# VladimirP1/rs-sync

Measured on AMD Instinct MI355X. Metric: ray-residuals/sec (PreSync sweep + Sync iter), 4096 frames x 2048 tracks, higher is better.
Workload: dtype f32

## Files before the change

### rs-sync_amd/csrc/kernels/sync64.hpp

```cpp
#pragma once

#pragma clang fp contract(off)

namespace {



struct Loss64Params {
    Rays64 rays;
    const FrameRec* frames;
    const uint32_t* sel;
    uint32_t n_sel;
    const d4* coef;
    int n_knots;
    double fs;
    const int32_t* kd;
    const double* fd;
    uint32_t n_delays;
    const uint32_t* grp;
    uint32_t n_grp;
    const double* M;
    const double* k;
    double* part_loss;
    double* part_grad;
// ... 462 lines not shown
            }
        } else {
        double ss = 0.0;
        if constexpr (RPT != 0) {
#pragma unroll
            for (int j = 0; j < RPT; ++j) {
                const double pm = p.simple_k ? sqrt(rs::dot(ev.P[j], ev.P[j])) : rs::dot(ev.P[j], Mv);
                ss = fma(pm, pm, ss);
            }
        } else {
            for (int j = 0; j < ev.rpt; ++j) {
                const size_t i = (size_t)j * kThreads + tid;
                const d3 Pj = d3{ev.gP[i], ev.gP[ev.g_rows + i], ev.gP[2 * (size_t)ev.g_rows + i]};
                const double pm = p.simple_k ? sqrt(rs::dot(Pj, Pj)) : rs::dot(Pj, Mv);
                ss = fma(pm, pm, ss);
            }
        }
        const double sw = wave_sum_f64(ss);
        if ((tid & 63) == 0) s_red[tid >> 6] = sw;
        __syncthreads();
        tot = s_red[0];
#pragma unroll
        for (int w = 1; w < NW; ++w) tot += s_red[w];
        }
        kk = clamp_k(100.0 / sqrt(tot));
        x[0] = Mv.x; x[1] = Mv.y; x[2] = Mv.z;
        if (tid == 0) {
            if (!p.simple_k) { st_m<SC1>(&p.M[3 * sf], x[0]); st_m<SC1>(&p.M[3 * sf + 1], x[1]); st_m<SC1>(&p.M[3 * sf + 2], x[2]); }
            st_m<SC1>(&p.k[sf], kk);
            if (p.init_h) st_m<SC1>(&p.init_h[sf], (int32_t)kInitNone);
        }
    } else {
        x[0] = m_x; x[1] = m_y; x[2] = m_z;
        kk = m_k;
    }
    if (mk_out) { mk_out[0] = x[0]; mk_out[1] = x[1]; mk_out[2] = x[2]; mk_out[3] = kk; }
    if (p.max_iters <= 0 || p.simple_k) return;
    ev.k2 = kk * kk;
    if constexpr (EMU4) {
        if ((size_t)N * 24u <= (size_t)p.win_bytes) {
            __syncthreads();
            __attribute__((address_space(3))) double* l = (__attribute__((address_space(3))) double*)reinterpret_cast<double*>(s_win);
            for (uint32_t row = tid; row < N; row += kThreads) {
                l[row] = ev.gP[row];
                l[N + row] = ev.gP[ev.g_rows + row];
                l[2 * N + row] = ev.gP[2 * (size_t)ev.g_rows + row];
            }
            __syncthreads();
            ev.lP = l;
            ev.n_lds = N;
        }
    }

    LbfgsHistLds hist{s_S, s_Y, s_inv_ys, s_rho, s_alpha};
    int best_not_last = 0;
    K3_T0();
    const int it = rs::lbfgs3(ev, hist, x, p.max_iters , p.reeval, &best_not_last);
    K3_ADD(12, 13);
    K3_FLUSH(ev);
    if (mk_out) { mk_out[0] = x[0]; mk_out[1] = x[1]; mk_out[2] = x[2]; }
    if (tid == 0) {
        st_m<SC1>(&p.M[3 * sf], x[0]); st_m<SC1>(&p.M[3 * sf + 1], x[1]); st_m<SC1>(&p.M[3 * sf + 2], x[2]);
        if (p.stats) {
            atomicAdd(&p.stats[0], (unsigned long long)it);
            atomicAdd(&p.stats[1], (unsigned long long)ev.evals);
            atomicAdd(&p.stats[2], (unsigned long long)best_not_last);
        }
        if (p.per_frame) {
            p.per_frame[2 * sf] = (uint32_t)it;
            p.per_frame[2 * sf + 1] = (uint32_t)ev.evals;
        }
        if (p.evals_out) p.evals_out[sf] = (uint32_t)ev.evals;
    }
}

template <int RPT, int NW>
__global__ __launch_bounds__(64 * NW, NW == 4 ? (RPT == 0 ? 2 : (RPT <= 8 ? 3 : (RPT <= 24 ? 2 : 1))) : (NW == 1 ? (RPT >= 8 ? 3 : 4) : 2)) void opt_motion64_kernel(Motion64Params p) {
    __shared__ MotionLds<NW> lds;
    extern __shared__ d4 s_motion_win[];
    opt_motion64_body<RPT, NW>(p, p.order ? p.order[blockIdx.x + p.slot0] : blockIdx.x + p.slot0, lds, s_motion_win, nullptr,
                               p.scratch0 + blockIdx.x);
}

__global__ __launch_bounds__(1024) void motion_order_kernel(const uint32_t* __restrict__ evals, const uint32_t* __restrict__ list,
                                                            uint32_t* __restrict__ order, uint32_t pos0, uint32_t count) {
    __shared__ uint32_t s_bin[256];
    for (uint32_t b = threadIdx.x; b < 256; b += blockDim.x) s_bin[b] = 0;
    __syncthreads();
    for (uint32_t i = threadIdx.x; i < count; i += blockDim.x) {
        const uint32_t e = evals[list[pos0 + i]];
        atomicAdd(&s_bin[e < 255u ? e : 255u], 1u);
    }
    __syncthreads();
    if (threadIdx.x == 0) {
        uint32_t at = 0;
        for (int b = 255; b >= 0; --b) {
            const uint32_t n = s_bin[b];
            s_bin[b] = at;
            at += n;
        }
    }
    __syncthreads();
    for (uint32_t i = threadIdx.x; i < count; i += blockDim.x) {
        const uint32_t s = list[pos0 + i];
        const uint32_t e = evals[s];
        const uint32_t pos = atomicAdd(&s_bin[e < 255u ? e : 255u], 1u);
        order[pos0 + pos] = s;
    }
}

struct Debug64Params {
    Rays64 rays;
    const FrameRec* frames;
    uint32_t fi;
    const d4* coef;
    int n_knots;
    double fs;
    int32_t kd;
    double fd;
    double* P;
    double* dP;
};

__global__ __launch_bounds__(kBlock) void debug_problem64_kernel(Debug64Params p) {
    __shared__ d4 s_win[4 * kWinMax];
    const FrameRec fr = p.frames[p.fi];
    Spline64 sp;
    sp.g = p.coef;
    sp.n = p.n_knots;
    sp.cap = kWinMax;
    sp.compact = 0;
    frame_window64(sp, s_win, fr, p.kd);
    __syncthreads();
    for (uint32_t row = blockIdx.x * kBlock + threadIdx.x; row < fr.n; row += gridDim.x * kBlock) {
        d3 P, dP;
        residual_row64<true>(sp, p.rays, (size_t)fr.off + row, fr.base_knot + p.kd, p.fd, P, dP);
        p.P[3 * row] = P.x; p.P[3 * row + 1] = P.y; p.P[3 * row + 2] = P.z;
        if (p.dP) { p.dP[3 * row] = dP.x * p.fs; p.dP[3 * row + 1] = dP.y * p.fs; p.dP[3 * row + 2] = dP.z * p.fs; }
    }
}

__global__ __launch_bounds__(64) void debug_math64_kernel(int op, const double* __restrict__ a, const double* __restrict__ b,
                                                          double* __restrict__ out, uint32_t n) {
    const uint32_t i = blockIdx.x * 64 + threadIdx.x;
    const double x = i < n ? a[i] : 0.0, y = (i < n && b) ? b[i] : 0.0;
    if (op == 4) {
        const double t = wave_sum_f64(x);
        if (threadIdx.x == 0) out[blockIdx.x] = t;
        return;
    }
    if (i >= n) return;
    if (op == 0) out[i] = x / y;
    else if (op == 1) out[i] = sqrt(x);
    else if (op == 2) { double rc; out[2 * i] = rs::log1p_rcp_f64(x, &rc); out[2 * i + 1] = rc; }
    else if (op == 5) out[i] = rs::div3_exact(x);
    else out[i] = fma(x, y, x);
}

}

#pragma clang fp contract(fast)
```

### rs-sync_amd/csrc/kernels/syncloop.hpp

```cpp
#pragma once

namespace {

constexpr int kMaxBt = 10, kHalfBt = 5;

struct SyncWin {
    double d, v;
    double x0;
    double l1, g1;
    int active, conv, hit, iters;
    int phase;
    int nf;
    int hit_prev;
};

struct SyncLoopParams {
    SyncWin* win;
    uint32_t n_win;
    uint32_t win0, win1;
    const double* part;
    uint32_t n_sel, rows;
    const uint32_t* chunk_off;
    const uint32_t* win_chunk_off;
    double* chunk_tmp;
    uint32_t chunk_stride;
    int32_t* mo_kd; double* mo_fd;
    int32_t* lg_kd; double* lg_fd;
    int32_t* tr_kd; double* tr_fd;
    double fs;
    double ts[11];
    double c_armijo, delay_b, search_center, search_radius;
    int it, max_outer;
    int nf_fixed;
    int nf_floor;
    double* ext_sums;
    int* n_active;
    double* trace;
};


__device__ __forceinline__ void split64_dev(double delay, double fs, int32_t* kd, double* fd) {
#pragma clang fp contract(off)
    if (delay != delay) { *kd = 0; *fd = delay; return; }
    const double D = delay * fs;
    const double kClamp = (double)(1 << 29);
    if (!(fabs(D) <= 1.79769313486231570e308)) { *kd = 0; *fd = 0.0; return; }
    const double fl = floor(D);
    if (fl > kClamp) { *kd = 1 << 29; *fd = 0.0; return; }
    if (fl < -kClamp) { *kd = -(1 << 29); *fd = 0.0; return; }
    *kd = (int32_t)fl;
    *fd = D - fl;
}

constexpr uint32_t kStageDoubles = 2048;
__device__ __forceinline__ void window_sums(const SyncLoopParams& p, uint32_t w, double* s_tot, double* s_stage) {
    const uint32_t c0 = p.win_chunk_off[w], c1 = p.win_chunk_off[w + 1], nc = c1 - c0;
    const uint32_t j_lo = p.chunk_off[c0], j_hi = p.chunk_off[c1], span = j_hi - j_lo;
    double* tmp = p.chunk_tmp + (size_t)w * (2 * kMaxBt) * p.chunk_stride;
    const bool staged = p.rows * span <= kStageDoubles;
    if (staged) {
        for (uint32_t e = threadIdx.x; e < p.rows * span; e += blockDim.x)
            s_stage[e] = p.part[(size_t)(e / span) * p.n_sel + j_lo + e % span];
        __syncthreads();
    }
    for (uint32_t e = threadIdx.x; e < p.rows * nc; e += blockDim.x) {
        const uint32_t r = e / nc, c = c0 + e % nc;
        double acc = 0.0;
        uint32_t j = p.chunk_off[c];
        const uint32_t j1 = p.chunk_off[c + 1];
        if (staged) {
            const double* row = s_stage + (size_t)r * span - j_lo;
            for (; j + 8 <= j1; j += 8) {
                double v[8];
#pragma unroll
                for (int q = 0; q < 8; ++q) v[q] = row[j + q];
#pragma unroll
                for (int q = 0; q < 8; ++q) acc += v[q];
            }
            for (; j < j1; ++j) acc += row[j];
        } else {
            const double* row = p.part + (size_t)r * p.n_sel;
            const uint32_t cnt = j1 - j;
            if (cnt <= 64) {
                double v[64];
#pragma unroll
                for (int q = 0; q < 64; ++q) v[q] = (uint32_t)q < cnt ? row[j + q] : 0.0;
#pragma unroll
                for (int q = 0; q < 64; ++q)
                    if ((uint32_t)q < cnt) acc += v[q];
            } else {
                for (; j < j1; ++j) acc += row[j];
            }
        }
        tmp[(size_t)r * p.chunk_stride + (c - c0)] = acc;
    }
    __syncthreads();
    for (uint32_t r = threadIdx.x; r < p.rows; r += blockDim.x) {
        const double* t = tmp + (size_t)r * p.chunk_stride;
        double acc = 0.0;
        uint32_t c = 0;
        for (; c + 16 <= nc; c += 16) {
            double v[16];
#pragma unroll
            for (int q = 0; q < 16; ++q) v[q] = t[c + q];
#pragma unroll
            for (int q = 0; q < 16; ++q) acc += v[q];
        }
        for (; c < nc; ++c) acc += t[c];
        s_tot[r] = acc;
    }
    __syncthreads();
}

__global__ __launch_bounds__(64) void sync_begin_kernel(SyncLoopParams p) {
#pragma clang fp contract(off)
    const uint32_t w = p.win0 + blockIdx.x * 64 + threadIdx.x;
    if (w >= p.win1) return;
    SyncWin& s = p.win[w];
    s.x0 = s.active ? s.d - p.delay_b * s.v : __builtin_nan("");
    split64_dev(s.active ? s.d : __builtin_nan(""), p.fs, &p.mo_kd[w], &p.mo_fd[w]);
    split64_dev(s.x0, p.fs, &p.lg_kd[w], &p.lg_fd[w]);
}

__device__ __forceinline__ bool trial_wanted(const SyncWin& s, int i) {
    if (!s.active) return false;
    return s.phase == 0 ? i < s.nf : i >= s.nf;
}

__device__ __forceinline__ void grad_decide(const SyncLoopParams& p, SyncWin& s, double l1, double g1) {
#pragma clang fp contract(off)
    if (s.active && s.phase == 0) {
        s.l1 = l1;
        s.g1 = g1;
        s.hit = -1;
        if (s.iters == 0 && !p.nf_fixed) {
            int i = 0;
            while (i < kMaxBt - 1 && p.ts[i] * fabs(s.g1) >= 1e-3) ++i;
            const int want = i + 2;
            s.nf = want < kHalfBt ? kHalfBt : (want > kMaxBt ? kMaxBt : want);
        }
    }
}
__device__ __forceinline__ void trial_delays(const SyncLoopParams& p, const SyncWin& s, int32_t* tr_kd, double* tr_fd, size_t stride) {
#pragma clang fp contract(off)
    for (int i = 0; i < kMaxBt; ++i) {
        const double td = trial_wanted(s, i) ? s.x0 - p.ts[i] * s.g1 : __builtin_nan("");
        split64_dev(td, p.fs, &tr_kd[(size_t)i * stride], &tr_fd[(size_t)i * stride]);
    }
}

__global__ __launch_bounds__(kBlock) void sync_sums_kernel(SyncLoopParams p) {
#pragma clang fp contract(off)
    __shared__ double s_tot[2 * kMaxBt];
    __shared__ double s_stage[kStageDoubles];
    const uint32_t w = blockIdx.x + p.win0;
    window_sums(p, w, s_tot, s_stage);
    for (uint32_t r = threadIdx.x; r < p.rows; r += blockDim.x) p.ext_sums[(size_t)r * p.n_win + w] = s_tot[r];
}
__device__ __forceinline__ void decision_sums(const SyncLoopParams& p, uint32_t w, double* s_tot, double* s_stage) {
    if (p.ext_sums) {
        for (uint32_t r = threadIdx.x; r < p.rows; r += blockDim.x) s_tot[r] = p.ext_sums[(size_t)r * p.n_win + w];
        __syncthreads();
    } else {
        window_sums(p, w, s_tot, s_stage);
    }
}

__global__ __launch_bounds__(kBlock) void sync_grad_kernel(SyncLoopParams p) {
#pragma clang fp contract(off)
    __shared__ double s_tot[2 * kMaxBt];
    __shared__ double s_stage[kStageDoubles];
    const uint32_t w = blockIdx.x + p.win0;
    decision_sums(p, w, s_tot, s_stage);
    if (threadIdx.x != 0) return;
    SyncWin& s = p.win[w];
    grad_decide(p, s, s_tot[0], s_tot[1]);
    trial_delays(p, s, p.tr_kd + w, p.tr_fd + w, p.n_win);
}

__device__ __forceinline__ void armijo(const SyncLoopParams& p, SyncWin& s, const double* lt, int b0, int b1) {
#pragma clang fp contract(off)
    if (!s.active || s.hit >= 0) return;
    const double m = s.g1 * s.g1;
    for (int i = b0; i < b1; ++i) {
        if (s.l1 - lt[i] >= p.ts[i] * p.c_armijo * m) {
            s.hit = i;
            break;
        }
    }
}

__device__ __forceinline__ bool step_decide(const SyncLoopParams& p, SyncWin& s, const double* lt, double* rows, size_t row_stride) {
#pragma clang fp contract(off)
    bool step_now = false;
    if (s.active) {
        if (s.phase == 0) {
            armijo(p, s, lt, 0, s.nf);
            if (s.hit >= 0 || s.nf >= kMaxBt) step_now = true;
            else s.phase = 1;
        } else {
            armijo(p, s, lt, s.nf, kMaxBt);
            step_now = true;
        }
    }
    if (step_now) {
        const double v = s.l1, g = s.g1;
        const double t = s.hit >= 0 ? p.ts[s.hit] : p.ts[kMaxBt];
        const int trials = s.hit >= 0 ? s.hit + 1 : kMaxBt;
        const double step = -t * g;
        s.v = p.delay_b * s.v + step;
        s.d += s.v;
        const double step_size = fabs(step);
        double* row = rows + (size_t)s.iters * row_stride;
        row[0] = s.d; row[1] = step; row[2] = v; row[3] = g; row[4] = t; row[5] = (double)trials;
        s.iters += 1;
        s.phase = 0;
        const int last = s.hit >= 0 ? s.hit : kMaxBt - 1;
        const int want = (last > s.hit_prev ? last : s.hit_prev) + 1;
        s.hit_prev = last;
        s.nf = p.nf_fixed ? p.nf_fixed : (want < p.nf_floor ? p.nf_floor : (want > kMaxBt ? kMaxBt : want));
        if (step_size < 1e-4) s.conv++; else s.conv = 0;
        bool stop = s.conv > 5;
        if (!stop && fabs(s.d - p.search_center) > p.search_radius) stop = true;
        if (stop || s.iters == p.max_outer) s.active = 0;
    }
    s.x0 = s.active ? s.d - p.delay_b * s.v : __builtin_nan("");
    return step_now;
}

__global__ __launch_bounds__(kBlock) void sync_step_kernel(SyncLoopParams p) {
#pragma clang fp contract(off)
    __shared__ double s_tot[2 * kMaxBt];
    __shared__ double s_stage[kStageDoubles];
    const uint32_t w = blockIdx.x + p.win0;
    decision_sums(p, w, s_tot, s_stage);
    if (threadIdx.x != 0) return;
    SyncWin& s = p.win[w];
    step_decide(p, s, s_tot, p.trace + (size_t)w * 6, (size_t)p.n_win * 6);
    if (s.active) atomicAdd(&p.n_active[p.it], 1);
    const bool go = s.active && s.phase == 0;
    split64_dev(go ? s.d : __builtin_nan(""), p.fs, &p.mo_kd[w], &p.mo_fd[w]);
    split64_dev(go ? s.x0 : __builtin_nan(""), p.fs, &p.lg_kd[w], &p.lg_fd[w]);
}

}
```

### rs-sync_amd/csrc/rssync_kernels.hip

```cpp
#include <hip/hip_runtime.h>

#include <dlfcn.h>

#include <algorithm>
#include <cmath>
#include <cstdio>
#include <cstdlib>
#include <cstring>
#include <mutex>
#include <string>
#include <thread>
#include <vector>

#ifndef RSSYNC_TEST_VARIANTS
#define RSSYNC_TEST_VARIANTS 0
#endif

#include "../../include/rssync_hip.h"
#include "track_hip.h"
#include "rectify_hip.h"
#include "stabilize_hip.h"
#include "color_hip.h"
#include "zoom_hip.h"
#include "limit_hip.h"
// ... 606 lines not shown
        p.slots = r.list;
        p.n_slots = r.count;
        p.chunk = wp.chunk;
        p.n_chunks = (p.n_cand + wp.chunk - 1) / wp.chunk;
        if (kind == LmedsKind::Small) {
            const uint32_t g1 = (uint32_t)((uint64_t)r.count * p.n_chunks);
            switch (rpt) {
                case 1: hipLaunchKernelGGL((lmeds_small_kernel<1, 0, 0, true>), dim3(g1), dim3(64), 0, c->stream, p); break;
                case 2: hipLaunchKernelGGL((lmeds_small_kernel<2, 0, 0, true>), dim3(g1), dim3(64), 0, c->stream, p); break;
                case 3: hipLaunchKernelGGL((lmeds_small_kernel<3, 0, 0, true>), dim3(g1), dim3(64), 0, c->stream, p); break;
                case 4: hipLaunchKernelGGL((lmeds_small_kernel<4, 0, 0, true>), dim3(g1), dim3(64), 0, c->stream, p); break;
                default: hipLaunchKernelGGL((lmeds_small_kernel<8, 0, 0, true>), dim3(g1), dim3(64), 0, c->stream, p); break;
            }
        } else {
            const uint32_t grid = (uint32_t)((uint64_t)((r.count + 7) / 8) * 8 * p.n_chunks);
            switch (rpt) {
                case 4: hipLaunchKernelGGL((lmeds_kernel<4, 0, 0, true, true>), dim3(grid), dim3(kBlock), 0, c->stream, p); break;
                case 8: hipLaunchKernelGGL((lmeds_kernel<8, 0, 0, true, true>), dim3(grid), dim3(kBlock), 0, c->stream, p); break;
                case 16: hipLaunchKernelGGL((lmeds_kernel<16, 0, 0, true, true>), dim3(grid), dim3(kBlock), 0, c->stream, p); break;
                case 24: allow_dynamic_lds(lmeds_kernel<24, 0, 0, true, true>, 0);
                         hipLaunchKernelGGL((lmeds_kernel<24, 0, 0, true, true>), dim3(grid), dim3(kBlock), 0, c->stream, p); break;
                case 32: allow_dynamic_lds(lmeds_kernel<16, 0, 0, true, true, kWideBlock>, 0);
                         hipLaunchKernelGGL((lmeds_kernel<16, 0, 0, true, true, kWideBlock>), dim3(grid), dim3(kWideBlock), 0, c->stream, p); break;
                default: return set_err(c, "lmeds (fp64 rows): unsupported rows-per-thread");
            }
        }
        RS_HIP(hipGetLastError());
    }
    return 0;
}

bool loss_fixed80(const rship_ctx* c, int k) {
    return c->cls_cap64[k] == (uint32_t)kWinMax && (class_span(c, k) + 1.f <= (float)kWinMax || c->force_general);
}
uint32_t loss_nb_run(const rship_ctx* c, int k) {
    return loss_fixed80(c, k) ? (uint32_t)kLossBatch : std::max(1u, std::min((uint32_t)kLossBatchWide, kLossWinBytes / (c->cls_cap64[k] * 128u)));
}

template <bool GRAD, bool SIMPLE>
int launch_loss64(rship_ctx* c, const Loss64Params& p_in, hipStream_t st = nullptr, uint32_t slot0 = 0, uint32_t count = 0) {
    if (!st) st = c->stream;
    ProfScope ps(c, GRAD ? RSHIP_K_LOSS_GRAD : RSHIP_K_LOSS);
    for (const ClassRange& r : class_ranges(c, slot0, count)) {
        Loss64Params p = p_in;
        const int k = r.k;
        p.slots = r.list;
        p.slot0 = r.list ? 0u : c->h_cls_slots[r.pos0];
        const uint32_t cap64 = cap64_of(c, k);
        p.win_cap = cap64;
        p.win_compact = compact_of(c, k) ? 1u : 0u;
        const bool fixed80 = !GRAD && loss_fixed80(c, k);
        p.nb_run = GRAD ? 1u : loss_nb_run(c, k);
        const size_t dyn = fixed80 ? 0 : (size_t)p.nb_run * cap64 * 128u, dyn_small = win64_bytes(c, k);
        if (k == 0 && !c->no_small_loss) {
            hipLaunchKernelGGL((loss64_small_kernel<GRAD, SIMPLE>), dim3(r.count), dim3(64), dyn_small, st, p);
            RS_HIP(hipGetLastError());
            continue;
        }
        const int rpt = k == 0 ? rpt_for(c->cls_max_n[0]) : class_rpt(c, k);
#define RS_LOSS_CASE(R)                                                                                                        \
    case R:                                                                                                                    \
        if constexpr (!GRAD) {                                                                                                 \
            if (fixed80) { hipLaunchKernelGGL((loss64_kernel<R, GRAD, SIMPLE, kWinMax>), dim3(r.count), dim3(kBlock), 0, st, p); break; } \
        }                                                                                                                      \
        hipLaunchKernelGGL((loss64_kernel<R, GRAD, SIMPLE, 0>), dim3(r.count), dim3(kBlock), dyn, st, p);                      \
        break;
        switch (rpt) {
            RS_LOSS_CASE(0)
            RS_LOSS_CASE(4)
            RS_LOSS_CASE(8)
            RS_LOSS_CASE(16)
            RS_LOSS_CASE(24)
            RS_LOSS_CASE(32)
            default: return set_err(c, "loss: unsupported rows-per-thread");
        }
#undef RS_LOSS_CASE
        RS_HIP(hipGetLastError());
    }
    return 0;
}

constexpr uint32_t kOrderMinSlots = 512;

int launch_motion64(rship_ctx* c, const Motion64Params& p_in, hipStream_t st = nullptr, uint32_t slot0 = 0, uint32_t count = 0) {
    if (!st) st = c->stream;
    ProfScope ps(c, RSHIP_K_MOTION);
    for (const ClassRange& r : class_ranges(c, slot0, count)) {
        Motion64Params p = p_in;
        const int k = r.k;
        p.slot0 = r.pos0;
        p.win_cap = cap64_of(c, k);
        p.win_compact = compact_of(c, k) ? 1u : 0u;
        const size_t dyn = win64_bytes(c, k);
        p.win_bytes = (uint32_t)dyn;
        const uint32_t cnt = r.count;
        if (k == 0) {
            const uint32_t n = c->cls_max_n[0];
            if (n <= 64) hipLaunchKernelGGL((opt_motion64_kernel<1, 1>), dim3(cnt), dim3(64), dyn, st, p);
            else if (n <= 128) hipLaunchKernelGGL((opt_motion64_kernel<2, 1>), dim3(cnt), dim3(64), dyn, st, p);
            else if (n <= 192) hipLaunchKernelGGL((opt_motion64_kernel<3, 1>), dim3(cnt), dim3(64), dyn, st, p);
            else if (n <= 256) hipLaunchKernelGGL((opt_motion64_kernel<4, 1>), dim3(cnt), dim3(64), dyn, st, p);
            else hipLaunchKernelGGL((opt_motion64_kernel<8, 1>), dim3(cnt), dim3(64), dyn, st, p);
        } else if (k == 1) hipLaunchKernelGGL((opt_motion64_kernel<4, 4>), dim3(cnt), dim3(256), dyn, st, p);
        else if (k == 2) hipLaunchKernelGGL((opt_motion64_kernel<8, 4>), dim3(cnt), dim3(256), dyn, st, p);
        else if (k == 3 && class_rpt(c, 3) == 16) hipLaunchKernelGGL((opt_motion64_kernel<16, 4>), dim3(cnt), dim3(256), dyn, st, p);
        else if (k == 3) hipLaunchKernelGGL((opt_motion64_kernel<24, 4>), dim3(cnt), dim3(256), dyn, st, p);
        else if (k == 4) hipLaunchKernelGGL((opt_motion64_kernel<32, 4>), dim3(cnt), dim3(256), dyn, st, p);
        else {
            if (!p.scratch || p.scratch_rows < c->cls_max_n[5]) return set_err(c, "motion: no scratch for frames of more than 8192 tracks");
            p.scratch0 = r.pos0 - c->cls_off[5];
            hipLaunchKernelGGL((opt_motion64_kernel<0, 4>), dim3(cnt), dim3(256), dyn, st, p);
        }
        RS_HIP(hipGetLastError());
        if (p.evals_out && p.order && c->mo_order.p && p.max_iters > 0 && !p.simple_k && cnt >= kOrderMinSlots) {
            hipLaunchKernelGGL(motion_order_kernel, dim3(1), dim3(1024), 0, st, (const uint32_t*)p.evals_out, (const uint32_t*)c->cls_slots.p,
                               (uint32_t*)c->mo_order.p, r.pos0, cnt);
            RS_HIP(hipGetLastError());
        }
    }
    return 0;
}

int launch_plan_sum(rship_ctx* c, const double* in, uint32_t rows, uint32_t cols, uint32_t slot = 0, uint32_t n_slots = 1) {
    if (!c->plan_wins) return set_err(c, "no reduction plan set");
    const size_t cs = (size_t)rows * (c->plan_chunks + 1), ws = (size_t)rows * c->plan_wins;
    if (n_slots > 1 && (c->chunk_out.cap < cs * n_slots * 8 || c->win_out.cap < ws * n_slots * 8)) return set_err(c, "plan sum: the batch's buffers were not sized");
    if (n_slots == 1 && (ensure(c, c->chunk_out, cs * 8) || ensure(c, c->win_out, ws * 8))) return 1;
    ProfScope ps(c, RSHIP_K_REDUCE);
    hipLaunchKernelGGL(plan_sum_kernel, dim3(rows * c->plan_wins), dim3(64), 0, c->stream, in, cols,
                       c->plan_has_idx ? (const uint32_t*)c->plan_idx.p : nullptr, (const uint32_t*)c->plan_chunk_off.p,
                       c->plan_chunks, (const uint32_t*)c->plan_win_off.p, c->plan_wins, (double*)c->chunk_out.p + cs * slot,
                       (double*)c->win_out.p + ws * slot);
    RS_HIP(hipGetLastError());
    return 0;
}

int queue_sums_to_host(rship_ctx* c, uint32_t rows, size_t at, size_t* off_chunk, size_t* end) {
    const size_t wb = (size_t)rows * c->plan_wins * 8, cb = (size_t)rows * c->plan_chunks * 8;
    if (ensure_pinned(c, at + wb + cb + 64)) return 1;
    RS_HIP(hipMemcpyAsync((char*)c->pinned + at, c->win_out.p, wb, hipMemcpyDeviceToHost, c->stream));
    if (cb) RS_HIP(hipMemcpyAsync((char*)c->pinned + at + wb, c->chunk_out.p, cb, hipMemcpyDeviceToHost, c->stream));
    *off_chunk = at + wb;
    *end = at + wb + cb;
    return 0;
}

struct DeviceGuard {
    int prev = -1;
    explicit DeviceGuard(const rship_ctx* c) {
        if (hipGetDevice(&prev) != hipSuccess) prev = -1;
        if (prev != c->device) (void)hipSetDevice(c->device);
        else prev = -1;
    }
    ~DeviceGuard() {
        if (prev >= 0) (void)hipSetDevice(prev);
    }
    DeviceGuard(const DeviceGuard&) = delete;
    DeviceGuard& operator=(const DeviceGuard&) = delete;
};

int upload_delays(rship_ctx* c, const int32_t* kd, const float* fd, size_t n) {
    if (ensure(c, c->kd, n * 8)) return 1;
    c->h_delays.resize(2 * n);
    memcpy(c->h_delays.data(), kd, n * 4);
    memcpy(c->h_delays.data() + n, fd, n * 4);
    RS_HIP(hipMemcpyAsync(c->kd.p, c->h_delays.data(), n * 8, hipMemcpyHostToDevice, c->stream));
    c->d_fd = (const float*)((const int32_t*)c->kd.p + n);
    return 0;
}
int upload_delays64(rship_ctx* c, const int32_t* kd, const double* fd, size_t n) {
    const size_t pad = (n + 1) / 2 * 2;
    if (ensure(c, c->kd64, pad * 4 + n * 8)) return 1;
    c->h_delays64.resize(pad + 2 * n);
    memcpy(c->h_delays64.data(), kd, n * 4);
    memcpy(c->h_delays64.data() + pad, fd, n * 8);
    RS_HIP(hipMemcpyAsync(c->kd64.p, c->h_delays64.data(), pad * 4 + n * 8, hipMemcpyHostToDevice, c->stream));
    c->d_fd64 = (const double*)((const int32_t*)c->kd64.p + pad);
    return 0;
}
Rays64 rays64_of(const rship_ctx* c) {
    const double2* q0 = (const double2*)c->rays64.p;
    const size_t tr = (size_t)c->total_rays;
    return Rays64{q0, q0 + tr, q0 + 2 * tr, q0 + 3 * tr};
}
int check_ready(rship_ctx* c) {
    if (!c->n_knots) return set_err(c, "no gyro spline uploaded");
    if (!c->n_frames) return set_err(c, "no frames uploaded");
    if (!c->n_sel) return set_err(c, "no frames selected");
    return 0;
}

}

namespace {
struct RcclId { char bytes[128]; };
using rccl_get_id_fn = int (*)(RcclId*);
using rccl_init_fn = int (*)(void**, int, RcclId, int);
// ... 1256 lines not shown
    size_t off = 0;
    auto take = [&](size_t bytes) { size_t o = off; off += (bytes + 255) / 256 * 256; return o; };
    const size_t o_win = take(W * sizeof(SyncWin));
    const size_t o_mokd = take(W * 4), o_mofd = take(W * 8), o_lgkd = take(W * 4), o_lgfd = take(W * 8);
    const size_t o_trkd = take((size_t)kMaxBt * W * 4), o_trfd = take((size_t)kMaxBt * W * 8);
    const size_t nact_stride = ((size_t)max_launch * 4 + 255) / 256 * 256;
    const size_t o_nact = take((size_t)G * nact_stride);
    const size_t o_trace = take((size_t)W * max_outer * 48);
    const size_t o_tmp = take((size_t)W * 2 * kMaxBt * (c->plan_max_chunks + 1) * 8);
    const size_t o_ext = take((size_t)2 * kMaxBt * W * 8);
    if (ensure(c, c->loop_state, off)) return 1;
    char* base = (char*)c->loop_state.p;
    if (ensure(c, c->part, (size_t)2 * kMaxBt * (ns + 1) * 8)) return 1;
    while (c->loop_streams.size() < G) {
        hipStream_t st = nullptr;
        RS_HIP(hipStreamCreateWithFlags(&st, hipStreamNonBlocking));
        c->loop_streams.push_back(st);
    }
    if (!c->loop_ready) RS_HIP(hipEventCreateWithFlags(&c->loop_ready, hipEventDisableTiming));

    std::vector<SyncWin> hw(W);
    for (uint32_t w = 0; w < W; ++w) {
        hw[w] = SyncWin{};
        hw[w].d = d0[w];
        hw[w].active = 1;
        hw[w].hit = -1;
        hw[w].nf = nf_fixed ? nf_fixed : nf_floor;
    }
    RS_HIP(hipMemcpyAsync(base + o_win, hw.data(), W * sizeof(SyncWin), hipMemcpyHostToDevice, c->stream));
    RS_HIP(hipMemsetAsync(base + o_nact, 0, (size_t)G * nact_stride, c->stream));

    SyncLoopParams lp{};
    lp.win = (SyncWin*)(base + o_win);
    lp.n_win = W;
    lp.part = (const double*)c->part.p;
    lp.n_sel = ns;
    lp.chunk_off = (const uint32_t*)c->plan_chunk_off.p;
    lp.win_chunk_off = (const uint32_t*)c->plan_win_off.p;
    lp.chunk_tmp = (double*)(base + o_tmp);
    lp.chunk_stride = c->plan_max_chunks + 1;
    lp.mo_kd = (int32_t*)(base + o_mokd); lp.mo_fd = (double*)(base + o_mofd);
    lp.lg_kd = (int32_t*)(base + o_lgkd); lp.lg_fd = (double*)(base + o_lgfd);
    lp.tr_kd = (int32_t*)(base + o_trkd); lp.tr_fd = (double*)(base + o_trfd);
    lp.fs = c->fs;
    {
        double t = 1e-3;
        for (int i = 0; i <= kMaxBt; ++i) { lp.ts[i] = t; t *= .1; }
    }
    lp.c_armijo = 2e-4;
    lp.delay_b = .3;
    lp.search_center = search_center;
    lp.search_radius = search_radius;
    lp.max_outer = max_outer;
    lp.nf_fixed = nf_fixed;
    lp.nf_floor = nf_floor;
    lp.trace = (double*)(base + o_trace);
    lp.ext_sums = ranked ? (double*)(base + o_ext) : nullptr;

    Motion64Params mp{};
    if (fill_motion(c, mp)) return 1;
    mp.kd = lp.mo_kd;
    mp.fd = lp.mo_fd;
    Loss64Params qp{};
    qp.rays = rays64_of(c);
    qp.frames = (const FrameRec*)c->frames.p;
    qp.sel = (const uint32_t*)c->sel.p;
    qp.n_sel = ns;
    qp.coef = (const d4*)c->coef64.p;
    qp.n_knots = (int)c->n_knots;
    qp.fs = c->fs;
    qp.grp = W > 1 ? (const uint32_t*)c->grp.p : nullptr;
    qp.n_grp = W;
    qp.M = (const double*)c->M.p;
    qp.k = (const double*)c->k.p;
    qp.part_loss = (double*)c->part.p;

    struct Group {
        uint32_t w0, w1, s0, s1;
        hipStream_t st;
        int* n_active;
        int* h_nact;
        int it = 0;
        bool done = false;
    };
    std::vector<Group> groups(G);
    if (ensure_pinned(c, (size_t)G * nact_stride + 64)) return 1;
    {
        uint32_t w = 0;
        for (uint32_t g = 0; g < G; ++g) {
            Group& gr = groups[g];
            gr.w0 = w;
            const uint64_t target = (uint64_t)ns * (g + 1) / G;
            while (w < W && (g + 1 == G || c->h_grp_off[w + 1] <= target || w == gr.w0)) ++w;
            if (g + 1 == G) w = W;
            gr.w1 = w;
            gr.s0 = c->h_grp_off[gr.w0];
            gr.s1 = c->h_grp_off[gr.w1];
            gr.st = G == 1 ? c->stream : c->loop_streams[g];
            gr.n_active = (int*)(base + o_nact + (size_t)g * nact_stride);
            gr.h_nact = (int*)((char*)c->pinned + (size_t)g * nact_stride);
            gr.done = gr.w1 == gr.w0;
        }
    }
    {
        std::vector<std::pair<uint32_t, uint32_t>> ranges;
        for (const Group& gr : groups)
            if (gr.s1 > gr.s0)
                for (const ClassRange& r : class_ranges(c, gr.s0, gr.s1 - gr.s0)) ranges.emplace_back(r.pos0, r.count);
        if (prepare_order(c, ranges)) return 1;
    }
    if (G > 1) {
        RS_HIP(hipEventRecord(c->loop_ready, c->stream));
        for (Group& gr : groups) RS_HIP(hipStreamWaitEvent(gr.st, c->loop_ready, 0));
    }
    auto enqueue_iteration = [&](Group& gr) -> int {
        SyncLoopParams l = lp;
        l.win0 = gr.w0; l.win1 = gr.w1;
        l.n_active = gr.n_active;
        l.it = gr.it;
        const uint32_t nw = gr.w1 - gr.w0, cnt = gr.s1 - gr.s0;
        const dim3 ctl_block(nw > 64 ? 64 : kBlock);
        Loss64Params q = qp;
        auto loss_launch = [&](bool grad) -> int {
            if (simplified) return grad ? launch_loss64<true, true>(c, q, gr.st, gr.s0, cnt) : launch_loss64<false, true>(c, q, gr.st, gr.s0, cnt);
            return grad ? launch_loss64<true, false>(c, q, gr.st, gr.s0, cnt) : launch_loss64<false, false>(c, q, gr.st, gr.s0, cnt);
        };
        if (gr.it == 0) {
            hipLaunchKernelGGL(sync_begin_kernel, dim3((nw + 63) / 64), dim3(64), 0, gr.st, l);
            RS_HIP(hipGetLastError());
        }
        if (!simplified && cnt) {
            if (launch_motion64(c, mp, gr.st, gr.s0, cnt)) return 1;
        }
        q.kd = l.lg_kd; q.fd = l.lg_fd; q.n_delays = 1;
        q.part_grad = q.part_loss + (size_t)ns;
        if (cnt && loss_launch(true)) return 1;
        l.rows = 2;
        auto exchange = [&](uint32_t rows) -> int {
            if (!ranked) return 0;
            hipLaunchKernelGGL(sync_sums_kernel, dim3(nw), ctl_block, 0, gr.st, l);
            RS_HIP(hipGetLastError());
            c->loop_exchanges += 1;
            if (c->loop_xchg) {
                xbuf.resize((size_t)rows * W);
                RS_HIP(hipMemcpyAsync(xbuf.data(), l.ext_sums, xbuf.size() * 8, hipMemcpyDeviceToHost, gr.st));
                RS_HIP(hipStreamSynchronize(gr.st));
                const int rc = c->loop_xchg(c->loop_xchg_user, xbuf.data(), xbuf.size());
                if (rc) return set_err(c, "sync_run: the loop's host exchange failed (" + std::to_string(rc) + ")");
                RS_HIP(hipMemcpyAsync(l.ext_sums, xbuf.data(), xbuf.size() * 8, hipMemcpyHostToDevice, gr.st));
                RS_HIP(hipStreamSynchronize(gr.st));
                return 0;
            }
            const int rc = allreduce(l.ext_sums, l.ext_sums, (size_t)rows * W,  8,  0, c->rccl_comm, gr.st);
            if (rc) return set_err(c, "rccl: ncclAllReduce failed (" + std::to_string(rc) + ")");
            return 0;
        };
        if (exchange(2)) return 1;
        {
            ProfScope ps(c, RSHIP_K_REDUCE);
            hipLaunchKernelGGL(sync_grad_kernel, dim3(nw), ctl_block, 0, gr.st, l);
        }
        q.kd = l.tr_kd; q.fd = l.tr_fd; q.n_delays = kMaxBt;
        q.part_grad = nullptr;
        l.rows = kMaxBt;
        if (cnt && loss_launch(false)) return 1;
        if (exchange(kMaxBt)) return 1;
        {
            ProfScope ps(c, RSHIP_K_REDUCE);
            hipLaunchKernelGGL(sync_step_kernel, dim3(nw), ctl_block, 0, gr.st, l);
        }
        RS_HIP(hipGetLastError());
        gr.it += 1;
        return 0;
    };

    const int kLook = 8;
    auto run_group = [&](Group& gr) -> int {
        DeviceGuard guard(c);
        while (!gr.done) {
            const int later = !ranked ? kLook / 2 : (c->loop_xchg ? 1 : 2);
            const int first = (ranked && c->loop_xchg) ? 1 : kLook;
            const int until = std::min(max_launch, gr.it + (gr.it == 0 ? first : later));
            while (gr.it < until)
                if (enqueue_iteration(gr)) return 1;
            RS_HIP(hipMemcpyAsync(gr.h_nact, gr.n_active, (size_t)gr.it * 4, hipMemcpyDeviceToHost, gr.st));
            RS_HIP(hipStreamSynchronize(gr.st));
            gr.done = gr.h_nact[gr.it - 1] == 0 || gr.it >= max_launch;
        }
        return 0;
    };
    {
        std::vector<std::thread> workers;
        std::vector<int> rc(G, 0);
        for (uint32_t g = 1; g < G; ++g) workers.emplace_back([&, g] { rc[g] = run_group(groups[g]); });
        rc[0] = run_group(groups[0]);
        for (std::thread& t : workers) t.join();
        for (uint32_t g = 0; g < G; ++g)
            if (rc[g]) return 1;
    }
    int it_max = 0;
    for (const Group& gr : groups) it_max = std::max(it_max, gr.it);
    it_max = std::min(it_max, max_outer);
    c->init_pending = false;
    if (G == 1) prof_collect(c);
    const size_t tr_bytes = (size_t)it_max * W * 48, win_bytes = W * sizeof(SyncWin);
    if (ensure_pinned(c, tr_bytes + win_bytes + 64)) return 1;
    RS_HIP(hipMemcpyAsync(c->pinned, base + o_win, win_bytes, hipMemcpyDeviceToHost, c->stream));
    RS_HIP(hipMemcpyAsync((char*)c->pinned + win_bytes, base + o_trace, tr_bytes, hipMemcpyDeviceToHost, c->stream));
    if (sync_stream(c)) return 1;
    memcpy(hw.data(), c->pinned, win_bytes);
    const double* tr = (const double*)((const char*)c->pinned + win_bytes);
    for (uint32_t w = 0; w < W; ++w) {
        d_out[w] = hw[w].d;
        iters[w] = hw[w].iters;
        for (int k = 0; k < hw[w].iters; ++k) memcpy(trace + ((size_t)w * max_outer + k) * 6, tr + ((size_t)k * W + w) * 6, 48);
    }
    return 0;
}

namespace {
size_t exec_region_bytes(rship_ctx* c) {
    uint32_t search_cap = 0;
    if (c->cls_off[1] != c->cls_off[0]) search_cap = plan_lmeds_window<1>(c, 0, 0.0, 1u).cap;
    size_t region = rs::exec_region_for(c->cls_cap64[0], compact_of(c, 0), search_cap);
    if (c->n_sel != c->cls_off[1] - c->cls_off[0]) region = std::max(region, (size_t)16 * 1024);
    for (int k = 1; k < 5; ++k)
        if (c->cls_off[k + 1] != c->cls_off[k]) {
            const WinPlan wp = plan_lmeds_window<1>(c, k, 0.0, 1u);
            region = std::max(region, (size_t)(wp.cap ? wp.cap : (uint32_t)kWinMax) * 64u);
        }
    return region;
}
}
int rship_exec_supported(rship_ctx* c) {
    if (c->force_big || !c->n_sel || c->n_sel >= (1u << 24)) return 0;
    for (uint32_t i : c->h_sel)
        if (c->h_frame_n[i] < 2) return 0;
    if (c->max_n > c->one_wave_max && c->max_n > c->exec_big_max) return 0;
    if (c->cls_off[5] != c->cls_off[4]) return 0;
    if ((uint64_t)(c->n_sel - (c->cls_off[1] - c->cls_off[0])) * c->exec_big_share > c->n_sel) return 0;
    return exec_region_bytes(c) <= 48u * 1024u ? 1 : 0;
}

int rship_sync_exec(rship_ctx* c, const double* d0, int repeats, uint32_t stream_first, uint32_t stream_stride, uint64_t seed,
                    int max_outer, double search_center, double search_radius, double* d_out, double* cost, int32_t* iters,
                    double* trace, uint32_t trace_rows) {
    DeviceGuard dev_guard(c);
    if (check_ready(c)) return 1;
    const uint32_t W = c->n_grp, ns = c->n_sel;
    if (!rship_exec_supported(c)) return set_err(c, "sync_exec: this selection is not for the executor (RSSYNC_FORCE_BIG, a frame of fewer than 2 tracks, a search window beyond a wave's LDS)");
    if (c->plan_wins != W || c->plan_has_idx || c->plan_len != ns) return set_err(c, "sync_exec: the plan must be the selection's groups");
    if (max_outer <= 0 || repeats < 1 || repeats > kExecMaxCalls) return set_err(c, "sync_exec: bad iteration or call count");
// ... 2149 lines not shown
```

Baseline: 139.3 billion.

## Tile long-window sync sums through LDS, mask unused rows, fuse motion ordering

Windows too long for the old LDS stage now use 1024-thread control blocks. These blocks stream chunk partials through a padded LDS tile with one wave per chunk and prefetch the next tile into registers. Trial rows the window will not use are masked out of the step reduction. The per-class motion ordering kernels are deferred into one extra block of sync_grad_kernel to save launches. In exchange the code gets more complexity and larger dynamic LDS, and the ordering now runs on a single block after the loss kernel instead of right after motion.

```diff
diff --git a/rs-sync_amd/csrc/kernels/sync64.hpp b/rs-sync_amd/csrc/kernels/sync64.hpp
--- a/rs-sync_amd/csrc/kernels/sync64.hpp
+++ b/rs-sync_amd/csrc/kernels/sync64.hpp
@@ -568,9 +568,9 @@
                                p.scratch0 + blockIdx.x);
 }
 
-__global__ __launch_bounds__(1024) void motion_order_kernel(const uint32_t* __restrict__ evals, const uint32_t* __restrict__ list,
-                                                            uint32_t* __restrict__ order, uint32_t pos0, uint32_t count) {
-    __shared__ uint32_t s_bin[256];
+__device__ __forceinline__ void motion_order_block(const uint32_t* __restrict__ evals, const uint32_t* __restrict__ list,
+                                                   uint32_t* __restrict__ order, uint32_t pos0, uint32_t count, uint32_t* s_bin) {
+    __syncthreads();
     for (uint32_t b = threadIdx.x; b < 256; b += blockDim.x) s_bin[b] = 0;
     __syncthreads();
     for (uint32_t i = threadIdx.x; i < count; i += blockDim.x) {
@@ -594,6 +594,19 @@
         order[pos0 + pos] = s;
     }
 }
+__global__ __launch_bounds__(1024) void motion_order_kernel(const uint32_t* __restrict__ evals, const uint32_t* __restrict__ list,
+                                                            uint32_t* __restrict__ order, uint32_t pos0, uint32_t count) {
+    __shared__ uint32_t s_bin[256];
+    motion_order_block(evals, list, order, pos0, count, s_bin);
+}
+constexpr int kOrderMaxJobs = 6;
+struct MotionOrderJobs {
+    const uint32_t* evals;
+    const uint32_t* list;
+    uint32_t* order;
+    uint32_t n;
+    uint32_t pos0[kOrderMaxJobs], count[kOrderMaxJobs];
+};
 
 struct Debug64Params {
     Rays64 rays;
diff --git a/rs-sync_amd/csrc/kernels/syncloop.hpp b/rs-sync_amd/csrc/kernels/syncloop.hpp
--- a/rs-sync_amd/csrc/kernels/syncloop.hpp
+++ b/rs-sync_amd/csrc/kernels/syncloop.hpp
@@ -24,6 +24,7 @@
     const uint32_t* win_chunk_off;
     double* chunk_tmp;
     uint32_t chunk_stride;
+    uint32_t stage_doubles;
     int32_t* mo_kd; double* mo_fd;
     int32_t* lg_kd; double* lg_fd;
     int32_t* tr_kd; double* tr_fd;
@@ -53,22 +54,34 @@
 }
 
 constexpr uint32_t kStageDoubles = 2048;
-__device__ __forceinline__ void window_sums(const SyncLoopParams& p, uint32_t w, double* s_tot, double* s_stage) {
+constexpr uint32_t kChunkSlots = 64;
+constexpr uint32_t kChunkPitch = kChunkSlots + 1;
+constexpr uint32_t kTileItems = 96, kTileLoads = 6;
+constexpr uint32_t kTileDoubles = kTileItems * kChunkPitch;
+constexpr uint32_t kChunkSumDoubles = 2 * kMaxBt * 64;
+constexpr uint32_t kOffCap = 1024;
+constexpr uint32_t kSumsLdsDoubles = kTileDoubles + kChunkSumDoubles + kOffCap / 2;
+static_assert(kSumsLdsDoubles * 8 + 2 * kMaxBt * 8 <= 65536, "a decision launch's LDS: the stage and s_tot");
+constexpr int kCtlBlockMax = 1024;
+static_assert(kTileDoubles >= kStageDoubles && kTileItems >= 2 * kMaxBt, "a tile holds the short windows' stage and at least one chunk of every row");
+
+__device__ __forceinline__ void window_sums(const SyncLoopParams& p, uint32_t w, uint32_t mask, double* s_tot, double* s_stage) {
     const uint32_t c0 = p.win_chunk_off[w], c1 = p.win_chunk_off[w + 1], nc = c1 - c0;
     const uint32_t j_lo = p.chunk_off[c0], j_hi = p.chunk_off[c1], span = j_hi - j_lo;
     double* tmp = p.chunk_tmp + (size_t)w * (2 * kMaxBt) * p.chunk_stride;
     const bool staged = p.rows * span <= kStageDoubles;
+    const double* sums = tmp;
+    uint32_t sums_pitch = p.chunk_stride;
     if (staged) {
+        mask = ~0u;
         for (uint32_t e = threadIdx.x; e < p.rows * span; e += blockDim.x)
             s_stage[e] = p.part[(size_t)(e / span) * p.n_sel + j_lo + e % span];
         __syncthreads();
-    }
-    for (uint32_t e = threadIdx.x; e < p.rows * nc; e += blockDim.x) {
-        const uint32_t r = e / nc, c = c0 + e % nc;
-        double acc = 0.0;
-        uint32_t j = p.chunk_off[c];
-        const uint32_t j1 = p.chunk_off[c + 1];
-        if (staged) {
+        for (uint32_t e = threadIdx.x; e < p.rows * nc; e += blockDim.x) {
+            const uint32_t r = e / nc, c = c0 + e % nc;
+            double acc = 0.0;
+            uint32_t j = p.chunk_off[c];
+            const uint32_t j1 = p.chunk_off[c + 1];
             const double* row = s_stage + (size_t)r * span - j_lo;
             for (; j + 8 <= j1; j += 8) {
                 double v[8];
@@ -78,39 +91,114 @@
                 for (int q = 0; q < 8; ++q) acc += v[q];
             }
             for (; j < j1; ++j) acc += row[j];
+            tmp[(size_t)r * p.chunk_stride + (c - c0)] = acc;
+        }
+    } else {
+        const uint32_t lane = threadIdx.x & 63u, n_waves = blockDim.x >> 6;
+        const uint32_t wave = (uint32_t)__builtin_amdgcn_readfirstlane((int)(threadIdx.x >> 6));
+        const uint32_t tile_items = n_waves * kTileLoads < kTileItems ? n_waves * kTileLoads : kTileItems;
+        const uint32_t tile_chunks = tile_items / p.rows;
+        if (p.stage_doubles < kSumsLdsDoubles || tile_chunks == 0) {
+            for (uint32_t e = threadIdx.x; e < p.rows * nc; e += blockDim.x) {
+                const uint32_t r = e / nc, c = c0 + e % nc;
+                if (!((mask >> r) & 1u)) continue;
+                const double* row = p.part + (size_t)r * p.n_sel;
+                double acc = 0.0;
+                for (uint32_t j = p.chunk_off[c]; j < p.chunk_off[c + 1]; ++j) acc += row[j];
+                tmp[(size_t)r * p.chunk_stride + (c - c0)] = acc;
+            }
         } else {
-            const double* row = p.part + (size_t)r * p.n_sel;
-            const uint32_t cnt = j1 - j;
-            if (cnt <= 64) {
-                double v[64];
-#pragma unroll
-                for (int q = 0; q < 64; ++q) v[q] = (uint32_t)q < cnt ? row[j + q] : 0.0;
-#pragma unroll
-                for (int q = 0; q < 64; ++q)
-                    if ((uint32_t)q < cnt) acc += v[q];
-            } else {
-                for (; j < j1; ++j) acc += row[j];
-            }
-        }
-        tmp[(size_t)r * p.chunk_stride + (c - c0)] = acc;
+            uint32_t* s_off = reinterpret_cast<uint32_t*>(s_stage + kTileDoubles + kChunkSumDoubles);
+            for (uint32_t i = threadIdx.x; i <= nc && i < kOffCap; i += blockDim.x) s_off[i] = p.chunk_off[c0 + i];
+            __syncthreads();
+            auto off = [&](uint32_t i) -> uint32_t { return i < kOffCap ? s_off[i] : p.chunk_off[c0 + i]; };
+            double* csum = tmp;
+            if (p.rows * nc <= kChunkSumDoubles) {
+                csum = s_stage + kTileDoubles;
+                sums_pitch = nc;
+            }
+            sums = csum;
+            double v[kTileLoads];
+            auto load_tile = [&](uint32_t ca) {
+                const uint32_t ntc = nc - ca < tile_chunks ? nc - ca : tile_chunks, items = p.rows * ntc;
+#pragma unroll
+                for (uint32_t q = 0; q < kTileLoads; ++q) {
+                    const uint32_t e = q * n_waves + wave, r = e / ntc, cl = ca + e % ntc;
+                    v[q] = 0.0;
+                    if (e < items && ((mask >> r) & 1u)) {
+                        const uint32_t j0 = off(cl);
+                        if (lane < off(cl + 1) - j0) v[q] = p.part[(size_t)r * p.n_sel + j0 + lane];
+                    }
+                }
+            };
+            load_tile(0);
+            for (uint32_t ca = 0; ca < nc; ca += tile_chunks) {
+                const uint32_t ntc = nc - ca < tile_chunks ? nc - ca : tile_chunks, items = p.rows * ntc;
+                const bool more = ca + tile_chunks < nc;
+#pragma unroll
+                for (uint32_t q = 0; q < kTileLoads; ++q) {
+                    const uint32_t e = q * n_waves + wave;
+                    if (e < items) s_stage[e * kChunkPitch + lane] = v[q];
+                }
+                __syncthreads();
+                if (more) load_tile(ca + tile_chunks);
+                for (uint32_t e = threadIdx.x; e < items; e += blockDim.x) {
+                    const uint32_t r = e / ntc, cl = ca + e % ntc;
+                    if (!((mask >> r) & 1u)) continue;
+                    const uint32_t j0 = off(cl), cnt = off(cl + 1) - j0;
+                    double acc = 0.0;
+                    if (cnt <= kChunkSlots) {
+                        const double* s = s_stage + e * kChunkPitch;
+                        double u[8], n[8];
+                        uint32_t i = 0;
+                        if (cnt >= 8) {
+#pragma unroll
+                            for (int q = 0; q < 8; ++q) u[q] = s[q];
+                        }
+                        for (; i + 8 <= cnt; i += 8) {
+                            const bool ahead = i + 16 <= cnt;
+                            if (ahead) {
+#pragma unroll
+                                for (int q = 0; q < 8; ++q) n[q] = s[i + 8 + q];
+                            }
+#pragma unroll
+                            for (int q = 0; q < 8; ++q) acc += u[q];
+                            if (ahead) {
+#pragma unroll
+                                for (int q = 0; q < 8; ++q) u[q] = n[q];
+                            }
+                        }
+                        for (; i < cnt; ++i) acc += s[i];
+                    } else {
+                        const double* row = p.part + (size_t)r * p.n_sel + j0;
+                        for (uint32_t i = 0; i < cnt; ++i) acc += row[i];
+                    }
+                    csum[(size_t)r * sums_pitch + cl] = acc;
+                }
+                if (more) __syncthreads();
+            }
+        }
     }
     __syncthreads();
     for (uint32_t r = threadIdx.x; r < p.rows; r += blockDim.x) {
-        const double* t = tmp + (size_t)r * p.chunk_stride;
+        const double* t = sums + (size_t)r * sums_pitch;
         double acc = 0.0;
         uint32_t c = 0;
-        for (; c + 16 <= nc; c += 16) {
-            double v[16];
-#pragma unroll
-            for (int q = 0; q < 16; ++q) v[q] = t[c + q];
-#pragma unroll
-            for (int q = 0; q < 16; ++q) acc += v[q];
-        }
-        for (; c < nc; ++c) acc += t[c];
+        if ((mask >> r) & 1u) {
+            for (; c + 16 <= nc; c += 16) {
+                double v[16];
+#pragma unroll
+                for (int q = 0; q < 16; ++q) v[q] = t[c + q];
+#pragma unroll
+                for (int q = 0; q < 16; ++q) acc += v[q];
+            }
+            for (; c < nc; ++c) acc += t[c];
+        }
         s_tot[r] = acc;
     }
     __syncthreads();
 }
+
 
 __global__ __launch_bounds__(64) void sync_begin_kernel(SyncLoopParams p) {
 #pragma clang fp contract(off)
@@ -125,6 +213,13 @@
 __device__ __forceinline__ bool trial_wanted(const SyncWin& s, int i) {
     if (!s.active) return false;
     return s.phase == 0 ? i < s.nf : i >= s.nf;
+}
+__device__ __forceinline__ uint32_t sums_row_mask(const SyncLoopParams& p, uint32_t w) {
+    if (p.rows != (uint32_t)kMaxBt) return ~0u;
+    const SyncWin s = p.win[w];
+    uint32_t mask = 0;
+    for (int i = 0; i < kMaxBt; ++i) mask |= trial_wanted(s, i) ? (1u << i) : 0u;
+    return mask;
 }
 
 __device__ __forceinline__ void grad_decide(const SyncLoopParams& p, SyncWin& s, double l1, double g1) {
@@ -149,12 +244,12 @@
     }
 }
 
-__global__ __launch_bounds__(kBlock) void sync_sums_kernel(SyncLoopParams p) {
+__global__ __launch_bounds__(kCtlBlockMax) void sync_sums_kernel(SyncLoopParams p) {
 #pragma clang fp contract(off)
     __shared__ double s_tot[2 * kMaxBt];
-    __shared__ double s_stage[kStageDoubles];
+    extern __shared__ double s_stage[];
     const uint32_t w = blockIdx.x + p.win0;
-    window_sums(p, w, s_tot, s_stage);
+    window_sums(p, w, sums_row_mask(p, w), s_tot, s_stage);
     for (uint32_t r = threadIdx.x; r < p.rows; r += blockDim.x) p.ext_sums[(size_t)r * p.n_win + w] = s_tot[r];
 }
 __device__ __forceinline__ void decision_sums(const SyncLoopParams& p, uint32_t w, double* s_tot, double* s_stage) {
@@ -162,14 +257,19 @@
         for (uint32_t r = threadIdx.x; r < p.rows; r += blockDim.x) s_tot[r] = p.ext_sums[(size_t)r * p.n_win + w];
         __syncthreads();
     } else {
-        window_sums(p, w, s_tot, s_stage);
-    }
-}
-
-__global__ __launch_bounds__(kBlock) void sync_grad_kernel(SyncLoopParams p) {
+        window_sums(p, w, sums_row_mask(p, w), s_tot, s_stage);
+    }
+}
+
+__global__ __launch_bounds__(kCtlBlockMax) void sync_grad_kernel(SyncLoopParams p, MotionOrderJobs order) {
 #pragma clang fp contract(off)
     __shared__ double s_tot[2 * kMaxBt];
-    __shared__ double s_stage[kStageDoubles];
+    extern __shared__ double s_stage[];
+    if (blockIdx.x >= p.win1 - p.win0) {
+        uint32_t* s_bin = reinterpret_cast<uint32_t*>(s_stage);
+        for (uint32_t i = 0; i < order.n; ++i) motion_order_block(order.evals, order.list, order.order, order.pos0[i], order.count[i], s_bin);
+        return;
+    }
     const uint32_t w = blockIdx.x + p.win0;
     decision_sums(p, w, s_tot, s_stage);
     if (threadIdx.x != 0) return;
@@ -228,10 +328,10 @@
     return step_now;
 }
 
-__global__ __launch_bounds__(kBlock) void sync_step_kernel(SyncLoopParams p) {
+__global__ __launch_bounds__(kCtlBlockMax) void sync_step_kernel(SyncLoopParams p) {
 #pragma clang fp contract(off)
     __shared__ double s_tot[2 * kMaxBt];
-    __shared__ double s_stage[kStageDoubles];
+    extern __shared__ double s_stage[];
     const uint32_t w = blockIdx.x + p.win0;
     decision_sums(p, w, s_tot, s_stage);
     if (threadIdx.x != 0) return;
diff --git a/rs-sync_amd/csrc/rssync_kernels.hip b/rs-sync_amd/csrc/rssync_kernels.hip
--- a/rs-sync_amd/csrc/rssync_kernels.hip
+++ b/rs-sync_amd/csrc/rssync_kernels.hip
@@ -712,7 +712,9 @@
 
 constexpr uint32_t kOrderMinSlots = 512;
 
-int launch_motion64(rship_ctx* c, const Motion64Params& p_in, hipStream_t st = nullptr, uint32_t slot0 = 0, uint32_t count = 0) {
+static_assert(kOrderMaxJobs >= kNumClasses, "one order range per size class");
+int launch_motion64(rship_ctx* c, const Motion64Params& p_in, hipStream_t st = nullptr, uint32_t slot0 = 0, uint32_t count = 0,
+                    MotionOrderJobs* defer = nullptr) {
     if (!st) st = c->stream;
     ProfScope ps(c, RSHIP_K_MOTION);
     for (const ClassRange& r : class_ranges(c, slot0, count)) {
@@ -743,6 +745,15 @@
         }
         RS_HIP(hipGetLastError());
         if (p.evals_out && p.order && c->mo_order.p && p.max_iters > 0 && !p.simple_k && cnt >= kOrderMinSlots) {
+            if (defer) {
+                defer->evals = (const uint32_t*)p.evals_out;
+                defer->list = (const uint32_t*)c->cls_slots.p;
+                defer->order = (uint32_t*)c->mo_order.p;
+                defer->pos0[defer->n] = r.pos0;
+                defer->count[defer->n] = cnt;
+                defer->n += 1;
+                continue;
+            }
             hipLaunchKernelGGL(motion_order_kernel, dim3(1), dim3(1024), 0, st, (const uint32_t*)p.evals_out, (const uint32_t*)c->cls_slots.p,
                                (uint32_t*)c->mo_order.p, r.pos0, cnt);
             RS_HIP(hipGetLastError());
@@ -2165,6 +2176,7 @@
         int* h_nact;
         int it = 0;
         bool done = false;
+        bool long_window = false;
     };
     std::vector<Group> groups(G);
     if (ensure_pinned(c, (size_t)G * nact_stride + 64)) return 1;
@@ -2183,6 +2195,8 @@
             gr.n_active = (int*)(base + o_nact + (size_t)g * nact_stride);
             gr.h_nact = (int*)((char*)c->pinned + (size_t)g * nact_stride);
             gr.done = gr.w1 == gr.w0;
+            for (uint32_t i = gr.w0; i < gr.w1; ++i)
+                gr.long_window = gr.long_window || (uint64_t)(c->h_grp_off[i + 1] - c->h_grp_off[i]) * (uint32_t)kMaxBt > kStageDoubles;
         }
     }
     {
@@ -2202,7 +2216,9 @@
         l.n_active = gr.n_active;
         l.it = gr.it;
         const uint32_t nw = gr.w1 - gr.w0, cnt = gr.s1 - gr.s0;
-        const dim3 ctl_block(nw > 64 ? 64 : kBlock);
+        const dim3 ctl_block(gr.long_window ? kCtlBlockMax : (nw > 64 ? 64 : kBlock));
+        l.stage_doubles = gr.long_window ? kSumsLdsDoubles : kStageDoubles;
+        const size_t ctl_lds = (size_t)l.stage_doubles * 8;
         Loss64Params q = qp;
         auto loss_launch = [&](bool grad) -> int {
             if (simplified) return grad ? launch_loss64<true, true>(c, q, gr.st, gr.s0, cnt) : launch_loss64<false, true>(c, q, gr.st, gr.s0, cnt);
@@ -2212,8 +2228,9 @@
             hipLaunchKernelGGL(sync_begin_kernel, dim3((nw + 63) / 64), dim3(64), 0, gr.st, l);
             RS_HIP(hipGetLastError());
         }
+        MotionOrderJobs order{};
         if (!simplified && cnt) {
-            if (launch_motion64(c, mp, gr.st, gr.s0, cnt)) return 1;
+            if (launch_motion64(c, mp, gr.st, gr.s0, cnt, ranked ? nullptr : &order)) return 1;
         }
         q.kd = l.lg_kd; q.fd = l.lg_fd; q.n_delays = 1;
         q.part_grad = q.part_loss + (size_t)ns;
@@ -2221,7 +2238,7 @@
         l.rows = 2;
         auto exchange = [&](uint32_t rows) -> int {
             if (!ranked) return 0;
-            hipLaunchKernelGGL(sync_sums_kernel, dim3(nw), ctl_block, 0, gr.st, l);
+            hipLaunchKernelGGL(sync_sums_kernel, dim3(nw), ctl_block, ctl_lds, gr.st, l);
             RS_HIP(hipGetLastError());
             c->loop_exchanges += 1;
             if (c->loop_xchg) {
@@ -2241,7 +2258,7 @@
         if (exchange(2)) return 1;
         {
             ProfScope ps(c, RSHIP_K_REDUCE);
-            hipLaunchKernelGGL(sync_grad_kernel, dim3(nw), ctl_block, 0, gr.st, l);
+            hipLaunchKernelGGL(sync_grad_kernel, dim3(nw + (order.n ? 1u : 0u)), ctl_block, ctl_lds, gr.st, l, order);
         }
         q.kd = l.tr_kd; q.fd = l.tr_fd; q.n_delays = kMaxBt;
         q.part_grad = nullptr;
@@ -2250,7 +2267,7 @@
         if (exchange(kMaxBt)) return 1;
         {
             ProfScope ps(c, RSHIP_K_REDUCE);
-            hipLaunchKernelGGL(sync_step_kernel, dim3(nw), ctl_block, 0, gr.st, l);
+            hipLaunchKernelGGL(sync_step_kernel, dim3(nw), ctl_block, ctl_lds, gr.st, l);
         }
         RS_HIP(hipGetLastError());
         gr.it += 1;
```

New measurement: 140.0 billion, median of 6. About the same (+0.5%).
